# luoao-kddi/SCP

Measured on AMD Instinct MI355X. Metric: KITTI frames/sec encode (SCP-EHEM, level 16) + bpp match vs ref, higher is better.
Workload: dtype f32 (dense layers and attention as bf16x3 split on bf16 MFMA, feature kNN as f16x3 split on f16 MFMA, fp32 accumulate; position kNN / CDF in fp32); 1 GPU; SCP-EHEM KITTI-like synthetic 120k-pt frames, --spher --mullevel lidar_level=16 (BASELINE.json configs[2]), seeded random weights; nodes_per_frame=577403, windows_per_frame=100, frames_per_gpu=46, frames_in_flight=4, frames_per_launch_sequence=1, transform=host-numpy on a prefetch thread (strict identity: the reference's integers), parallelism=frame-sharded x1, rank_cores=256, rank_cores_pinned=False

## Files before the change

### include/scp_debug.h

```cpp
#ifndef SCP_DEBUG_H
#define SCP_DEBUG_H
#include "scp.h"

#ifdef __cplusplus
extern "C" {
#endif

SCP_API int scp_set_knn_mode(int32_t f16x3);
SCP_API int scp_set_attention_mode(int32_t bf16x3);

SCP_API int scp_set_knn_workgroup(int32_t shape);
SCP_API int scp_knn_debug_buffer(unsigned long long *dev_buf);
SCP_API int scp_rc_debug_buffer(unsigned long long *dev_buf);
SCP_API int scp_set_attention_variant(int32_t v);
SCP_API int scp_get_attention_variant(void);
SCP_API int scp_rc_set_grid(int32_t workgroups);
SCP_API int scp_rc_set_wide(int32_t mode);

enum {
    SCP_PROF_POST_ATTN = 1,
    SCP_PROF_LN_LINEAR = 2,
    SCP_PROF_ATTENTION = 3,
    SCP_PROF_KNN_FEAT = 4,
    SCP_PROF_KNN_POS = 5,
    SCP_PROF_GEMM_SPLIT = 6,
    SCP_PROF_EDGE_MLP = 7,
    SCP_PROF_MERGE = 8,
    SCP_PROF_EDGE_GATHER = 9,
    SCP_PROF_CDF = 10,
    SCP_PROF_GEMM_F32 = 11,
    SCP_PROF_GEMM_ROWS = 12,
    SCP_PROF_SPLIT_ROWS = 13,
    SCP_PROF_LAYERNORM = 14,
    SCP_PROF_OA_ATTENTION = 15,
    SCP_PROF_GEOM = 16,
    SCP_PROF_OTHER = 17,
    SCP_PROF_MLP3 = 18,
    SCP_PROF_RATE = 19,
    SCP_PROF_NTAGS = 20
};
SCP_API int scp_prof_enable(int32_t on);
SCP_API int scp_prof_count(void);
SCP_API int scp_prof_read(int32_t cap, int32_t *tags, float *ms, double *work);

#ifdef __cplusplus
// ... 4 lines not shown
```

### scp_amd/csrc/gemm_split.hip

```cpp
#include <stdlib.h>
#include "scp_internal.h"

typedef __bf16 bf16x8 __attribute__((ext_vector_type(8)));
typedef __bf16 bf16x4 __attribute__((ext_vector_type(4)));
typedef _Float16 sf16x8 __attribute__((ext_vector_type(8)));
typedef float f32x16 __attribute__((ext_vector_type(16)));
typedef float f32x4 __attribute__((ext_vector_type(4)));

enum { ACT_NONE = 0, ACT_LEAKY = 1, ACT_GELU = 2, ACT_RELU = 3 };

template <int act>
__device__ __forceinline__ float apply_act_s(float y) {
    if (act == ACT_LEAKY) return y > 0.f ? y : 0.01f * y;
    if (act == ACT_GELU) return scp_gelu(y);
    if (act == ACT_RELU) return y > 0.f ? y : 0.f;
    return y;
}

typedef __attribute__((address_space(3))) void *lds_ptr_t;
typedef const __attribute__((address_space(1))) void *glb_ptr_t;

__device__ __forceinline__ void dma16(const void *g, char *l) {
    __builtin_amdgcn_global_load_lds((glb_ptr_t)g, (lds_ptr_t)l, 16, 0, 0);
}
// ... 567 lines not shown
    const int64_t blk = i >> 6;
    const int nks = Kpad >> 5;
    const int ks = (int)(blk % nks);
    const int64_t rb = blk / nks;
    const int q = p ^ ((r >> 2) & 3);
    dst[i] = src[((rb * 16 + r) * (int64_t)Kpad + 32 * ks + 8 * q) >> 3];
}

extern "C" SCP_API int scp_tile_weight_bf16(const void *plane, int32_t Npad, int32_t Kpad, void *tiled, void *stream) {
    if (!plane || !tiled || Npad <= 0 || Kpad <= 0 || (Npad & 15) || (Kpad & 31) || (((uintptr_t)plane | (uintptr_t)tiled) & 15)) return SCP_EINVAL;
    const int64_t total = (int64_t)Npad * Kpad / 8;
    hipLaunchKernelGGL(tile_weight_kernel, dim3((unsigned)cdiv64(total, 256)), dim3(256), 0, (hipStream_t)stream, (const uint4 *)plane, Npad, Kpad, (uint4 *)tiled);
    LAUNCH_CHECK();
    return SCP_OK;
}

extern "C" SCP_API int scp_split_rows(const float *src, int64_t ld_src, int64_t n_src, const int64_t *idx, int32_t C, void *hi, void *lo,
                                      int64_t ldo, int64_t rows, void *stream) {
    if (!src || !hi || !lo || rows < 0 || C <= 0 || (C & 3) || (ld_src & 3) || (ldo & 7) || ldo < C || (((uintptr_t)src) & 15) ||
        (((uintptr_t)hi | (uintptr_t)lo) & 7))
        return SCP_EINVAL;
    if (rows == 0) return SCP_OK;
    int Cp = (C + 31) & ~31;
    if (Cp > ldo) Cp = C;
    const int64_t total = rows * (Cp / 4);
    SCP_PROF(SCP_PROF_SPLIT_ROWS, stream, 8.0 * rows * C);
    hipLaunchKernelGGL(split_rows_kernel, dim3((unsigned)cdiv64(total, 256)), dim3(256), 0, (hipStream_t)stream, src, ld_src, n_src, idx, C / 4,
                       Cp / 4, (__bf16 *)hi, (__bf16 *)lo, ldo, total);
    LAUNCH_CHECK();
    return SCP_OK;
}

static int g_num_cu = 0;
template <int WM, int WN, int TM, bool EXT, bool F16 = false>
static int launch_cfg(const GemmSplitArgs &ga, int act, hipStream_t st, double work) {
    constexpr int BM = WM * TM * 32, BN = WN * 64;
    constexpr int STAGE = (BM + BN) * 128;
    constexpr int BOUNCE = WM * WN * 8192;
    constexpr int LDS = STAGE + (STAGE > BOUNCE ? STAGE : BOUNCE) + (EXT ? 2 * BM * 8 : 0);
    static bool configured = false;
    if (!configured) {
        HIP_TRY(hipFuncSetAttribute((const void *)gemm_split_kernel<WM, WN, TM, ACT_NONE, EXT, F16>, hipFuncAttributeMaxDynamicSharedMemorySize, LDS));
        HIP_TRY(hipFuncSetAttribute((const void *)gemm_split_kernel<WM, WN, TM, ACT_RELU, EXT, F16>, hipFuncAttributeMaxDynamicSharedMemorySize, LDS));
        if (!F16) {
            HIP_TRY(hipFuncSetAttribute((const void *)gemm_split_kernel<WM, WN, TM, ACT_LEAKY, EXT, false>, hipFuncAttributeMaxDynamicSharedMemorySize, LDS));
            HIP_TRY(hipFuncSetAttribute((const void *)gemm_split_kernel<WM, WN, TM, ACT_GELU, EXT, false>, hipFuncAttributeMaxDynamicSharedMemorySize, LDS));
        }
        configured = true;
    }
    const int64_t ntiles = cdiv64(ga.M, BM) * cdiv64(ga.N, BN);
    const int64_t slots = (int64_t)g_num_cu * (WM * WN == 4 ? 2 : 1);
    const unsigned grid = (unsigned)(ntiles < slots ? ntiles : slots);
    SCP_PROF(SCP_PROF_GEMM_SPLIT, st, work);
#define GOS(ACT, F) hipLaunchKernelGGL((gemm_split_kernel<WM, WN, TM, ACT, EXT, F>), dim3(grid), dim3(WM * WN * 64), LDS, st, ga)
    if (F16) { if (act == ACT_RELU) GOS(ACT_RELU, F16); else GOS(ACT_NONE, F16); }
    else switch (act) { case ACT_LEAKY: GOS(ACT_LEAKY, false); break; case ACT_GELU: GOS(ACT_GELU, false); break; case ACT_RELU: GOS(ACT_RELU, false); break; default: GOS(ACT_NONE, false); }
#undef GOS
    LAUNCH_CHECK();
    return SCP_OK;
}

static int linear_split_impl(const void *Ahi, const void *Alo, int64_t lda, const void *Whi, const void *Wlo, int32_t Npad, int32_t Kpad,
                             const float *bias, const float *residual, int64_t ldr, const int64_t *res_map, int32_t res_first, const int64_t *out_map, float *C, int64_t ldc,
                             void *Ohi, void *Olo, int64_t ldo, int32_t M, int32_t N, int32_t K, int32_t act, int32_t cfg, void *stream) {
    if (!Ahi || !Alo || !Whi || !Wlo || (!C && !Ohi) || ((Ohi == nullptr) != (Olo == nullptr)) || M <= 0 || N <= 0 || K <= 0 || (lda & 7) ||
        Kpad < K || (Kpad & 31) || lda < Kpad || (Npad & 255) || Npad < N || act < 0 || act > 3 || (C && ldc < N) ||
// ... 1 lines not shown
        (((uintptr_t)Ahi | (uintptr_t)Alo | (uintptr_t)Whi | (uintptr_t)Wlo) & 15) || (((uintptr_t)C | (uintptr_t)residual) & 3) ||
        (((uintptr_t)Ohi | (uintptr_t)Olo) & 7))
        return SCP_EINVAL;
    if (!g_num_cu) {
        int dev = 0;
        hipDeviceProp_t p;
        HIP_TRY(hipGetDevice(&dev));
        HIP_TRY(hipGetDeviceProperties(&p, dev));
        g_num_cu = p.multiProcessorCount > 0 ? p.multiProcessorCount : 256;
    }
    GemmSplitArgs ga;
    ga.a_isc = nullptr; ga.w_isc = nullptr; ga.row_max = nullptr; ga.col_max = nullptr; ga.cm_lo = ga.cm_hi = ga.cm_rows = 0;
    ga.Ahi = (const __bf16 *)Ahi; ga.Alo = (const __bf16 *)Alo; ga.lda = lda;
    ga.Whi = (const __bf16 *)Whi; ga.Wlo = (const __bf16 *)Wlo; ga.Kpad = Kpad;
    ga.bias = bias; ga.res = residual; ga.ldr = ldr; ga.C = C; ga.ldc = ldc;
    ga.res_map = residual ? res_map : nullptr; ga.res_first = (residual && res_first) ? 1 : 0;
    ga.out_map = C ? out_map : nullptr;
    ga.Ohi = (__bf16 *)Ohi; ga.Olo = (__bf16 *)Olo; ga.ldo = ldo; ga.M = M; ga.N = N;
    int nco = (N + 31) & ~31;
    if (nco > ldo) nco = (N + 3) & ~3;
    ga.ncols_out = nco;
    { static int wt = -1; if (wt < 0) { const char *e = getenv("SCP_WTILE"); wt = (e && e[0] == '0') ? 0 : 1; } ga.wtiled = wt; }
    if (cfg & ~0xff) {
        static int probe = -1;
        if (probe < 0) probe = getenv("SCP_GEMM_PROBE") ? 1 : 0;
        if (!probe || (cfg & ~0x300ff)) return SCP_EINVAL;
        if (cfg & 0x10000) ga.lda = 0;
        if (cfg & 0x20000) { ga.C = nullptr; ga.Ohi = ga.Olo = nullptr; ga.res = nullptr; }
    }
    cfg &= 255;
    ga.vec_ok = !((C && ((ldc & 3) || ((uintptr_t)C & 15))) || (residual && ((ldr & 3) || ((uintptr_t)residual & 15))));
    hipStream_t st = (hipStream_t)stream;
    const bool ext = ga.res_map || ga.res_first || ga.out_map;
    if (cfg == 0) {
        cfg = (N <= 128) ? 2 : 1;
        static int small = -1;
        if (small < 0) { const char *e = getenv("SCP_GEMM_SMALL"); small = (e && e[0] == '0') ? 0 : 1; }
        if (small && cdiv64(M, 256) * cdiv64(N, 256) * 2 <= g_num_cu) cfg = ext ? 2 : 3;
    }
    const double work = 2.0 * M * (double)N * K;
    if (cfg == 2) return ext ? launch_cfg<4, 2, 2, true>(ga, act, st, work) : launch_cfg<4, 2, 2, false>(ga, act, st, work);
    if (cfg == 3) return ext ? SCP_EINVAL : launch_cfg<2, 2, 2, false>(ga, act, st, work);
    return ext ? launch_cfg<2, 4, 4, true>(ga, act, st, work) : launch_cfg<2, 4, 4, false>(ga, act, st, work);
}

extern "C" SCP_API int scp_linear_split(const void *Ahi, const void *Alo, int64_t lda, const void *Whi, const void *Wlo, int32_t Npad, int32_t Kpad,
                                        const float *bias, const float *residual, int64_t ldr, float *C, int64_t ldc, void *Ohi, void *Olo,
                                        int64_t ldo, int32_t M, int32_t N, int32_t K, int32_t act, int32_t cfg, void *stream) {
    return linear_split_impl(Ahi, Alo, lda, Whi, Wlo, Npad, Kpad, bias, residual, ldr, nullptr, 0, nullptr, C, ldc, Ohi, Olo, ldo, M, N, K, act, cfg, stream);
}

static int linear_split_f16_impl(const void *Ahi, const void *Alo, int64_t lda, const float *a_inv_scale, const void *Whi, const void *Wlo,
                                 const float *w_inv_scale, int32_t Npad, int32_t Kpad, const float *bias, const float *residual, int64_t ldr,
                                 float *C, int64_t ldc, int32_t M, int32_t N, int32_t K, int32_t act, int32_t cfg, uint32_t *row_max, uint32_t *col_max,
                                 int32_t col_lo, int32_t col_hi, int32_t col_rows, void *stream) {
    if (col_max && (col_lo < 0 || col_hi > N || col_lo >= col_hi || col_rows <= 0)) return SCP_EINVAL;
    if ((((uintptr_t)row_max | (uintptr_t)col_max) & 3)) return SCP_EINVAL;
    if (!Ahi || !Alo || !a_inv_scale || !Whi || !Wlo || !w_inv_scale || !C || M <= 0 || N <= 0 || K <= 0 || (lda & 7) || Kpad < K || (Kpad & 31) || cfg < 0 || cfg > 3 ||
        lda < Kpad || (Npad & 255) || Npad < N || (act != ACT_NONE && act != ACT_RELU) || ldc < N || (residual && ldr < N) ||
        (((uintptr_t)Ahi | (uintptr_t)Alo | (uintptr_t)Whi | (uintptr_t)Wlo) & 15) || (((uintptr_t)C | (uintptr_t)residual) & 3))
        return SCP_EINVAL;
    if (!g_num_cu) {
        int dev = 0;
        hipDeviceProp_t p;
        HIP_TRY(hipGetDevice(&dev));
        HIP_TRY(hipGetDeviceProperties(&p, dev));
        g_num_cu = p.multiProcessorCount > 0 ? p.multiProcessorCount : 256;
    }
    GemmSplitArgs ga = {};
    ga.Ahi = (const __bf16 *)Ahi; ga.Alo = (const __bf16 *)Alo; ga.lda = lda;
    ga.Whi = (const __bf16 *)Whi; ga.Wlo = (const __bf16 *)Wlo; ga.Kpad = Kpad;
    ga.bias = bias; ga.res = residual; ga.ldr = ldr; ga.C = C; ga.ldc = ldc; ga.M = M; ga.N = N;
    ga.a_isc = a_inv_scale; ga.w_isc = w_inv_scale;
// ... 82 lines not shown
```

### scp_amd/csrc/knn.hip

```cpp
#include <float.h>
#include <stdlib.h>
#include <limits.h>
#include "scp_internal.h"

#define TK 20
typedef float f32x4 __attribute__((ext_vector_type(4)));
typedef float f32x16 __attribute__((ext_vector_type(16)));

__device__ __forceinline__ void topk_insert(float (&v)[TK], int (&id)[TK], float d, int j) {
#pragma unroll
    for (int t = 0; t < TK; ++t) {
        const bool better = (d > v[t]) || (d == v[t] && j < id[t]);
        const float nv = better ? d : v[t], od = better ? v[t] : d;
        const int ni = better ? j : id[t], oj = better ? id[t] : j;
        v[t] = nv; d = od; id[t] = ni; j = oj;
    }
}

__global__ __launch_bounds__(256) void sqnorm_kernel(const float *__restrict__ x, int64_t npts, int C, float *__restrict__ xx) {
    const int64_t i = (int64_t)blockIdx.x * 256 + threadIdx.x;
    if (i >= npts) return;
    const float *p = x + i * C;
    float s = 0.f;
    for (int c = 0; c < C; ++c) s = s + p[c] * p[c];
// ... 404 lines not shown
        if (s + 2 < nt) { nxt = next_tile(); issue(nxt, (s + 2) % NST); }
        const char *arow = pool + buf * STAGE_B + col * RB;
        f32x16 acc;
#pragma unroll
        for (int r = 0; r < 16; ++r) acc[r] = 0.f;
        f16x8 ca = *(const f16x8 *)(arow + 16 * ((0 + h) ^ swz));
        f16x8 cb = *(const f16x8 *)(arow + 16 * ((K / 8 + h) ^ swz));
        __builtin_amdgcn_sched_group_barrier(0x100, 2, 0);
#pragma unroll
        for (int c = 0; c < NC; ++c) {
            f16x8 na = ca, nb = cb;
            if (c + 1 < NC) {
                na = *(const f16x8 *)(arow + 16 * ((2 * (c + 1) + h) ^ swz));
                nb = *(const f16x8 *)(arow + 16 * ((K / 8 + 2 * (c + 1) + h) ^ swz));
            }
            acc = __builtin_amdgcn_mfma_f32_32x32x16_f16(cb, qa[c], acc, 0, 0, 0);
            acc = __builtin_amdgcn_mfma_f32_32x32x16_f16(ca, qb[c], acc, 0, 0, 0);
            acc = __builtin_amdgcn_mfma_f32_32x32x16_f16(ca, qa[c], acc, 0, 0, 0);
            ca = na; cb = nb;
            if (c + 1 < NC) __builtin_amdgcn_sched_group_barrier(0x100, 2, 0);
            __builtin_amdgcn_sched_group_barrier(0x008, 3, 0);
        }
        const float *sxx = txx + buf * 64;
        knn_select<true>(acc, sxx, sxx + 32, 2.f * isq, xxi, cur * 32, n, h, key, thr0v);
        cur = cur1;
        cur1 = nxt;
    }
    __syncthreads();
    knn_merge_write(key, (float *)pool, (int *)(pool + 128 * 2 * TK * 4), tid, w, col, h, q0, n, k, row0, ctab, idx);
}

struct KnnWg { int32_t row0, n, q0, pad; };

__global__ __launch_bounds__(1024) void knn_sched_kernel(const int *__restrict__ ctab, int nchunks, KnnWg *__restrict__ tab, int nslots, int nspill, int nsplit) {
    __shared__ int seq_base[2048], seq_n[2048], seq_blk0[2049];
    __shared__ unsigned long long seq_w0[2049];
    __shared__ int nseq_s, first_blk[9], spill_s;
    __shared__ unsigned long long wtot_s;
    const int tid = threadIdx.x;
    if (tid == 0) { nseq_s = 0; spill_s = 0; }
    if (tid < 9) first_blk[tid] = INT_MAX;
    __syncthreads();
    if (tid < 64) {
        int cnt = 0;
        for (int g = 0; g < nchunks; g += 64) {
            const int c = g + tid;
            const bool st = c < nchunks && ctab[2 * c] == c * 512 && ctab[2 * c + 1] > 0;
            const unsigned long long m = __ballot(st);
            if (st) {
                const int o = cnt + __popcll(m & ((1ull << tid) - 1ull));
                if (o < 2048) { seq_base[o] = ctab[2 * c]; seq_n[o] = ctab[2 * c + 1]; }
            }
            cnt += __popcll(m);
        }
        if (tid == 0) nseq_s = cnt < 2048 ? cnt : 2048;
    }
    __syncthreads();
    const int nseq = nseq_s;
    if (tid == 0) {
        int b = 0;
        unsigned long long wsum = 0;
        for (int q = 0; q < nseq; ++q) {
            seq_blk0[q] = b; seq_w0[q] = wsum;
            const int nb = ((seq_n[q] + 255) >> 8) * nsplit;
            b += nb; wsum += (unsigned long long)nb * (unsigned)(seq_n[q] / nsplit + 1);
        }
        seq_blk0[nseq] = b; seq_w0[nseq] = wsum; wtot_s = wsum ? wsum : 1ull;
    }
    __syncthreads();
    const int nblk = seq_blk0[nseq];
    const unsigned long long wtot = wtot_s;
    auto xcd_of = [&](int q, int j) { const unsigned long long cw = seq_w0[q] + (unsigned long long)j * (unsigned)(seq_n[q] / nsplit + 1); const int x = (int)(cw * 8ull / wtot); return x > 7 ? 7 : x; };
    for (int q = tid; q < nseq; q += 1024) {
        const int nb = seq_blk0[q + 1] - seq_blk0[q];
        for (int j = 0; j < nb; ++j) atomicMin(&first_blk[xcd_of(q, j)], seq_blk0[q] + j);
    }
    __syncthreads();
    for (int q = tid; q < nseq; q += 1024) {
        const int nb = seq_blk0[q + 1] - seq_blk0[q];
        for (int j = 0; j < nb; ++j) {
            const int x = xcd_of(q, j), slot = seq_blk0[q] + j - first_blk[x];
            KnnWg e; e.row0 = seq_base[q]; e.n = seq_n[q]; e.q0 = (j / nsplit) * 256; e.pad = j % nsplit;
            if (slot < nslots) tab[slot * 8 + x] = e;
            else { const int k = atomicAdd(&spill_s, 1); if (k < nspill) tab[nslots * 8 + k] = e; }
        }
    }
    (void)nblk;
}

template <int K, int G, bool DBG = false>
__global__ __launch_bounds__(512, 2) void knn_f16x3_wg256_kernel(const _Float16 *__restrict__ planes, const float *__restrict__ xx,
                                                                const float *__restrict__ inv_scale, const KnnWg *__restrict__ tab,
                                                                int *__restrict__ idx, const float *__restrict__ thr0, int order,
                                                                unsigned long long *__restrict__ dbg = nullptr, int nsplit = 1,
                                                                float *__restrict__ pval = nullptr, int *__restrict__ pidx = nullptr,
                                                                int64_t prows = 0) {
    constexpr int RB = 4 * K;
    constexpr int R = RB / 16;
    constexpr int NC = K / 16;
    constexpr int STAGE_B = 32 * RB;
    constexpr int NDMA = STAGE_B / 1024;
    constexpr int NDMA_W = (NDMA + 7) / 8;
    constexpr int NST = 2 * G;
    constexpr int NXX = NST;
    constexpr int MERGE_B = 2 * 256 * 2 * TK * 4;
    constexpr int TILES_B = NST * STAGE_B + NXX * 64 * 4;
    constexpr int POOL_B = TILES_B > MERGE_B ? TILES_B : MERGE_B;
    static_assert(STAGE_B % 1024 == 0 && POOL_B <= 160 * 1024, "layout");
    __shared__ __attribute__((aligned(1024))) char pool[POOL_B];
    float *txx = (float *)(pool + NST * STAGE_B);

    const KnnWg wg = tab[blockIdx.x];
    const int n = wg.n;
    if (n <= 0) return;
    const int tid = threadIdx.x, lane = tid & 63, col = lane & 31, h = lane >> 5;
    const int w = __builtin_amdgcn_readfirstlane(tid >> 6);
    const size_t row0 = (size_t)wg.row0;
    const int q0 = wg.q0;
    const char *pb = (const char *)planes + row0 * RB;
    const float *xxb = xx + row0, *isb = inv_scale + row0;
// ... 332 lines not shown

struct KnnScratch { void *stream; bool used; unsigned long long last; DevBuf buf; };
static KnnScratch g_xx_tab[8];
static unsigned long long g_xx_clock = 0;
static DevBuf *knn_scratch(hipStream_t st) {
    ++g_xx_clock;
    for (auto &e : g_xx_tab) if (e.used && e.stream == (void *)st) { e.last = g_xx_clock; return &e.buf; }
    KnnScratch *pick = nullptr;
    for (auto &e : g_xx_tab) if (!e.used) { pick = &e; break; }
    if (!pick) {
        for (auto &e : g_xx_tab) if (!pick || e.last < pick->last) pick = &e;
        pick->buf.release();
    }
    pick->used = true; pick->stream = (void *)st; pick->last = g_xx_clock;
    return &pick->buf;
}

static int g_knn_mode = -1;
static int knn_mode() {
    const int c = scp_ctx_knn_mode();
    if (c >= 0) return c;
    if (g_knn_mode < 0) { const char *e = getenv("SCP_KNN"); g_knn_mode = (e && e[0] == 'f') ? 0 : 1; }
    return g_knn_mode;
}
extern "C" SCP_API int scp_set_knn_mode(int32_t f16x3) { g_knn_mode = f16x3 ? 1 : 0; return SCP_OK; }
static int knn_split_on() {
    static int on = -1;
    if (on < 0) { const char *e = getenv("SCP_KNN_SPLIT"); on = (e && e[0] == '0') ? 0 : 1; }
    return on;
}
static int g_knn_wg = -1;
static int knn_wg() { if (g_knn_wg < 0) { const char *e = getenv("SCP_KNN_WG"); g_knn_wg = e ? atoi(e) : 256; } return g_knn_wg; }
extern "C" SCP_API int scp_set_knn_workgroup(int32_t v) { g_knn_wg = v; return SCP_OK; }

static int knn_launch(const float *x, int64_t npts, int C, dim3 grid, int n, int k, int *idx, const int *ctab, hipStream_t st,
                      const float *thr0 = nullptr) {
    const size_t xx_bytes = ((size_t)npts * sizeof(float) + 1023) & ~(size_t)1023;
    const bool split = (C == 144 || C == 192) && knn_mode() == 1;
    const int RB = C * 4;
    DevBuf *sp = knn_scratch(st);
    if (!sp) return SCP_EINVAL;
    DevBuf &sbuf = *sp;
    int nsplit = 1;
    if (split && ctab && knn_wg() == 256 && !g_knn_dbg && knn_split_on()) {
        const int64_t nblk = npts / 256 > 0 ? npts / 256 : 1;
        while (nsplit < 16 && nblk * (nsplit * 2) <= 256 && npts / 32 >= 8 * (int64_t)nsplit) nsplit *= 2;
    }
    const size_t part_bytes = nsplit > 1 ? (size_t)nsplit * (size_t)npts * TK * 8 + 256 : 0;
    int rc = sbuf.reserve(xx_bytes * (split ? 2 : 1) + (C <= 4 ? (size_t)npts * 16 + ((size_t)npts / 32 + grid.y + 1) * 32 : (split ? (size_t)npts * RB + 256 + (((size_t)(npts / 256) * 2 + 8) * nsplit + 520) * sizeof(KnnWg) + part_bytes : 0)));
    if (rc) return rc;
    float *xx = sbuf.as<float>();
    void *aux = (char *)sbuf.p + xx_bytes;
    if (split) {
        float *isc = (float *)aux;
        _Float16 *pl = (_Float16 *)((char *)aux + xx_bytes);
        hipLaunchKernelGGL(split2_kernel, dim3((unsigned)cdiv64(npts, 64)), dim3(256), 0, st, x, npts, C, pl, xx, isc);
        if (ctab && knn_wg() >= 256 && npts / 512 <= 2048) {
            const int nchunks = (int)(npts / 512);
            const int nspill = (int)(npts / 256) * nsplit;
            const int nslots = nspill / 8 + 64;
            const int nblocks = nslots * 8 + nspill;
            KnnWg *tab = (KnnWg *)((char *)pl + (((size_t)npts * RB + 255) & ~(size_t)255));
            float *pval = (float *)((char *)tab + (((size_t)nblocks * sizeof(KnnWg) + 255) & ~(size_t)255));
            int *pidx = (int *)(pval + (size_t)nsplit * (size_t)npts * TK);
            HIP_TRY(hipMemsetAsync(tab, 0, (size_t)nblocks * sizeof(KnnWg), st));
            hipLaunchKernelGGL(knn_sched_kernel, dim3(1), dim3(1024), 0, st, ctab, nchunks, tab, nslots, nspill, nsplit);
            const int shape = knn_wg() & 15, order = (knn_wg() >> 4) & 7;
            SCP_PROF(SCP_PROF_KNN_FEAT, st, (double)C);
#define KNN_LAUNCH(KK, GG) hipLaunchKernelGGL((knn_f16x3_wg256_kernel<KK, GG>), dim3(nblocks), dim3(512), 0, st, (const _Float16 *)pl, (const float *)xx, \
                                              (const float *)isc, (const KnnWg *)tab, idx, thr0, order, (unsigned long long *)nullptr, nsplit, pval, pidx, (int64_t)npts)
            if (C == 144) { if (shape == 2) KNN_LAUNCH(144, 1); else if (shape == 1) KNN_LAUNCH(144, 2); else KNN_LAUNCH(144, 4); }
            else if (g_knn_dbg && shape == 0)
                hipLaunchKernelGGL((knn_f16x3_wg256_kernel<192, 3, true>), dim3(nblocks), dim3(512), 0, st, (const _Float16 *)pl, (const float *)xx,
                                   (const float *)isc, (const KnnWg *)tab, idx, thr0, order, g_knn_dbg);
            else { if (shape == 2) KNN_LAUNCH(192, 1); else if (shape == 1) KNN_LAUNCH(192, 2); else KNN_LAUNCH(192, 3); }
#undef KNN_LAUNCH
            LAUNCH_CHECK();
            if (nsplit > 1) {
                hipLaunchKernelGGL(knn_merge_split_kernel, dim3((unsigned)cdiv64(npts, 256)), dim3(256), 0, st, ctab, (const float *)pval, (const int *)pidx, (int64_t)npts, nsplit, idx);
                LAUNCH_CHECK();
            }
            return SCP_OK;
        }
        SCP_PROF(SCP_PROF_KNN_FEAT, st, (double)C);
        if (C == 144) hipLaunchKernelGGL(knn_f16x3_kernel<144>, grid, dim3(256), 0, st, (const _Float16 *)pl, (const float *)xx, (const float *)isc, n, k, idx, ctab, thr0);
        else hipLaunchKernelGGL(knn_f16x3_kernel<192>, grid, dim3(256), 0, st, (const _Float16 *)pl, (const float *)xx, (const float *)isc, n, k, idx, ctab, thr0);
        LAUNCH_CHECK();
        return SCP_OK;
    }
    hipLaunchKernelGGL(sqnorm_kernel, dim3((unsigned)cdiv64(npts, 256)), dim3(256), 0, st, x, npts, C, xx);
    if (C <= 4) {
        hipLaunchKernelGGL(pad4_kernel, dim3((unsigned)cdiv64(npts, 256)), dim3(256), 0, st, x, npts, C, (float *)aux);
        float *bb = (float *)((char *)aux + (size_t)npts * 16);
        const int bn = ctab ? (int)npts : n, bB = ctab ? 1 : (int)grid.y;
        hipLaunchKernelGGL(bbox32_kernel, dim3((unsigned)cdiv64((int64_t)((bn + 31) / 32) * bB, 256)), dim3(256), 0, st, (const float *)aux, bn, bB, bb);
        SCP_PROF(SCP_PROF_KNN_POS, st, 4.0);
        hipLaunchKernelGGL((knn_mfma_kernel<2, 16, true>), grid, dim3(256), 0, st, (const float *)aux, (const float *)xx, n, 4, k, idx, ctab, thr0,
                           (const float *)bb);
    } else {
// ... 53 lines not shown
```

### scp_amd/native.py

```python
import ctypes as C
import os

import numpy as np
import torch

HERE = os.path.dirname(os.path.abspath(__file__))
LIB_PATH = os.path.join(HERE, "libscp_hip.so")
MAX_DEPTH = 21

CART, SPHER, CYLIN = 0, 1, 2
POS_MINMAX, POS_MINMAX_MUL, POS_POW2 = 0, 1, 2
_ERR = {-1: "SCP_EINVAL", -2: "SCP_ENOMEM", -3: "SCP_ESMALL", -4: "SCP_EHIP", -5: "SCP_ESTATE"}


class ScpError(RuntimeError):
    pass


class QuantInfo(C.Structure):
    _fields_ = [("bin_num", C.c_double), ("qs", C.c_double * 3), ("offset", C.c_double * 3),
                ("max_coord", C.c_int32), ("min_coord", C.c_int32)]


class Segment(C.Structure):
# ... 45 lines not shown
        "scp_geom_emit_nodes": (C.c_int, [_vp, _vp, _vp, _vp, _vp, _vp, _vp]),
        "scp_geom_emit_leaves": (C.c_int, [_vp, i32, _vp, _vp]),
        "scp_geom_krecords_i64": (C.c_int, [_vp, i32, _vp, _vp]),
        "scp_geom_context_ehem": (C.c_int, [_vp, i32, i32, i32, _vp, _vp, _vp, _vp, _vp]),
        "scp_geom_context_octattn": (C.c_int, [_vp, i32, _vp, _vp, _vp, _vp]),
        "scp_knn_topk": (C.c_int, [_vp, i32, i32, i32, i32, _vp, _vp]),
        "scp_knn_topk_packed": (C.c_int, [_vp, _vp, i32, i32, _vp, _vp]),
        "scp_knn_topk_packed_bounded": (C.c_int, [_vp, _vp, i32, i32, _vp, _vp, _vp]),
        "scp_swin_attention_packed": (C.c_int, [_vp, _vp, _vp, _vp, _vp, i32, i32, i32, i32, _vp, _vp]),
        "scp_swin_attention_packed_split": (C.c_int, [_vp, _vp, _vp, _vp, _vp, i32, i32, i32, i32, _vp, _vp, i64, _vp]),
        "scp_set_attention_mode": (C.c_int, [i32]),
        "scp_set_attention_variant": (C.c_int, [i32]),
        "scp_get_attention_variant": (C.c_int, []),
        "scp_ctx_create": (C.c_int, [C.POINTER(_vp)]),
        "scp_ctx_destroy": (C.c_int, [_vp]),
        "scp_ctx_set": (C.c_int, [_vp, i32, i32]),
        "scp_ctx_get": (C.c_int, [_vp, i32]),
        "scp_ctx_make_current": (C.c_int, [_vp]),
        "scp_rc_debug_buffer": (C.c_int, [_vp]),
        "scp_rc_set_wide": (C.c_int, [i32]),
        "scp_prof_enable": (C.c_int, [i32]),
        "scp_prof_count": (C.c_int, []),
        "scp_prof_read": (C.c_int, [i32, _vp, _vp, _vp]),
        "scp_set_knn_mode": (C.c_int, [i32]),
        "scp_row_scale_f16": (C.c_int, [_vp, i64, i32, i32, _vp, _vp, _vp]),
        "scp_row_scale_from_max": (C.c_int, [_vp, i32, _vp, _vp, _vp]),
        "scp_linear_split_f16_max": (C.c_int, [_vp, _vp, i64, _vp, _vp, _vp, _vp, i32, i32, _vp, _vp, i64, _vp, i64, i32, i32, i32, i32, i32, _vp, _vp, i32, i32, i32, _vp]),
        "scp_octattn_attention_f16x3_vmax": (C.c_int, [_vp, _vp, _vp, _vp, _vp, i64, i32, i32, i32, i32, _vp, _vp, _vp, i64, _vp, _vp]),
        "scp_linear_f16x3_scaled": (C.c_int, [_vp, i64, _vp, _vp, _vp, i32, _vp, _vp, i64, _vp, i64, i32, i32, i32, i32, _vp, _vp, _vp]),
        "scp_layernorm_add": (C.c_int, [_vp, _vp, i64, i32, _vp, _vp, C.c_float, _vp, _vp]),
        "scp_layernorm_add_split_f16": (C.c_int, [_vp, _vp, i64, i32, _vp, _vp, C.c_float, _vp, _vp, _vp, i64, _vp, _vp, _vp]),
        "scp_set_knn_workgroup": (C.c_int, [i32]),
        "scp_knn_debug_buffer": (C.c_int, [_vp]),
        "scp_nn_sqdist_f64": (C.c_int, [_vp, i64, _vp, i64, _vp, _vp]),
        "scp_estimate_normals_f64": (C.c_int, [_vp, i64, C.c_double, i32, _vp, _vp, _vp, _vp, _vp]),
        "scp_nn_tieset_f64": (C.c_int, [i32, _vp, i64, _vp, i64, _vp, _vp, _vp, _vp]),
        "scp_edge_gather_max_ld": (C.c_int, [_vp, i64, _vp, i64, _vp, _vp, _vp, i32, i32, i32, i32, _vp, i32, _vp]),
        "scp_embed_gather": (C.c_int, [_vp, _vp, _vp, i64, _vp, _vp, _vp, _vp, _vp, _vp, i64, _vp]),
        "scp_packed_plan_sizes": (C.c_int, [_vp, i32, _vp]),
        "scp_packed_plan": (C.c_int, [_vp, i32, _vp, _vp, i32, _vp]),
        "scp_decode_expand": (C.c_int, [_vp, _vp, _vp, _vp, _vp, i64, i32, i32, i32, i32, i32, C.c_double, C.c_double, _vp, _vp, _vp, _vp, _vp, _vp, _vp]),
        "scp_edge_gather_max": (C.c_int, [_vp, _vp, _vp, _vp, _vp, i32, i32, i32, i32, _vp, i32, _vp]),
        "scp_swin_attention": (C.c_int, [_vp, _vp, _vp, _vp, i32, i32, i32, i32, i32, _vp, _vp]),
        "scp_octattn_attention": (C.c_int, [_vp, _vp, _vp, _vp, _vp, i32, i32, i32, i32, _vp, _vp, _vp]),
        "scp_octattn_f16x3_ws_bytes": (C.c_int64, [i32, i32, i32]),
        "scp_octattn_embed": (C.c_int, [_vp, _vp, i64, i32, _vp, i32, _vp, i32, i32, _vp, i32, _vp, _vp, i32, _vp, i32, _vp, _vp, _vp, i64, _vp, _vp, _vp]),
        "scp_octattn_attention_f16x3": (C.c_int, [_vp, _vp, _vp, _vp, _vp, i64, i32, i32, i32, i32, _vp, _vp, _vp, i64, _vp]),
        "scp_octattn_attention_rowinv": (C.c_int, [_vp, i64, i64, _vp, _vp, i64, i64, _vp, _vp, i64, i64, _vp, _vp, i64, i64, i32, i32, i32, i32, i32,
                                                   i32, _vp]),
        "scp_octattn_attention_rowinv_step": (C.c_int, [_vp, i64, _vp, _vp, i64, i64, i32, i32, _vp, _vp, i64, _vp, _vp, i64, _vp, _vp, i32, i32, i32,
                                                        _vp]),
        "scp_decode_expand_octattn": (C.c_int, [_vp, _vp, _vp, _vp, i64, i32, i32, i32, _vp, _vp, _vp, _vp, _vp]),
        "scp_decode_expand_batch": (C.c_int, [_vp, _vp, _vp, _vp, _vp, i64, _vp, i32, i32, _vp, i32, i64, i64, _vp, _vp, _vp, _vp, _vp, _vp, _vp, _vp]),
        "scp_split_weight_bf16": (C.c_int, [_vp, i32, i32, i32, i32, _vp, _vp, _vp]),
        "scp_linear_bf16x3": (C.c_int, [_vp, i64, _vp, _vp, i32, _vp, _vp, i64, _vp, i64, i32, i32, i32, i32, _vp]),
        "scp_split_weight_f16": (C.c_int, [_vp, i32, i32, i32, i32, _vp, _vp, _vp, _vp]),
        "scp_linear_f16x3": (C.c_int, [_vp, i64, _vp, _vp, _vp, i32, _vp, _vp, i64, _vp, i64, i32, i32, i32, i32, _vp, _vp]),
        "scp_linear_split": (C.c_int, [_vp, _vp, i64, _vp, _vp, i32, i32, _vp, _vp, i64, _vp, i64, _vp, _vp, i64, i32, i32, i32, i32, i32, _vp]),
        "scp_tile_weight_bf16": (C.c_int, [_vp, i32, i32, _vp, _vp]),
        "scp_swin_ln_linear": (C.c_int, [_vp, i64, _vp, _vp, _vp, _vp, _vp, C.c_float, _vp, i64, i32, i32, _vp]),
        "scp_swin_post_attn": (C.c_int, [_vp, _vp, i64, _vp, i64, _vp, _vp, _vp, _vp, C.c_float, _vp, i64, i32, _vp, i32, _vp]),
        "scp_swin_post_attn_weight_bytes": (C.c_int64, []),
        "scp_gelu_prescale": (C.c_double, []),
        "scp_split_rows": (C.c_int, [_vp, i64, i64, _vp, i32, _vp, _vp, i64, i64, _vp]),
        "scp_linear_split_scatter": (C.c_int, [_vp, _vp, i64, _vp, _vp, i32, i32, _vp, _vp, _vp, i64, i32, i32, i32, i32, i32, _vp]),
        "scp_linear_split_gather": (C.c_int, [_vp, _vp, i64, _vp, _vp, i32, i32, _vp, _vp, i64, _vp, _vp, i64, _vp, _vp, i64, i32, i32, i32, i32, i32, _vp]),
# ... 483 lines not shown
            L = (L + 1) // 2
        return out
    parts = lists(e, n_self) + lists(e // 2, n_cross)
    flat = torch.from_numpy(np.concatenate(parts)).to(device, non_blocking=True)
    cuts = np.cumsum([0] + [len(p) for p in parts])
    views = [flat[cuts[i]:cuts[i + 1]] for i in range(len(parts))]
    return views[:n_self], views[n_self:]


def edge_gather_max_rows(u, v, idx, scale, shift, out=None):
    n, Co = u.shape
    if out is None:
        out = torch.empty((n, Co), dtype=torch.float32, device=u.device)
    elif out.shape != (n, Co) or out.stride(1) != 1 or out.dtype != torch.float32 or out.stride(0) % 4 or out.data_ptr() % 16:
        raise ScpError("edge_gather_max_rows: out must be a float32 [n, C'] view with unit channel stride and 16-byte aligned rows")
    _check(lib().scp_edge_gather_max_ld(u.data_ptr(), u.stride(0), v.data_ptr(), v.stride(0), _dev(idx, torch.int32), _dev(scale), _dev(shift),
                                        1, n, Co, idx.shape[1], out.data_ptr(), out.stride(0), _stream()), "scp_edge_gather_max_ld")
    return out


_MODES = {"knn": "f32" if os.environ.get("SCP_KNN", "")[:1] == "f" else "f16x3",
          "attn": "f32" if os.environ.get("SCP_ATTN", "")[:1] == "f" else "bf16x3"}


def set_knn_mode(f16x3):
    _check(lib().scp_set_knn_mode(1 if f16x3 else 0), "scp_set_knn_mode")
    _MODES["knn"] = "f16x3" if f16x3 else "f32"


def set_knn_workgroup(shape):
    _check(lib().scp_set_knn_workgroup(int(shape)), "scp_set_knn_workgroup")


class NumericProfile:

    def __init__(self, knn_f16x3=True, attention_bf16x3=True):
        self._h = _vp()
        _check(lib().scp_ctx_create(C.byref(self._h)), "scp_ctx_create")
        self.knn_f16x3, self.attention_bf16x3 = bool(knn_f16x3), bool(attention_bf16x3)
        _check(lib().scp_ctx_set(self._h, 1, int(self.knn_f16x3)), "scp_ctx_set")
        _check(lib().scp_ctx_set(self._h, 2, int(self.attention_bf16x3)), "scp_ctx_set")

    def describe(self, model_name):
        return numeric_profile(model_name, self)

    def __del__(self):
        try:
            if self._h:
                lib().scp_ctx_destroy(self._h)
        except Exception:
            pass


_TLS = __import__("threading").local()


def current_profile():
    return getattr(_TLS, "profile", None)


class use_profile:

    def __init__(self, profile):
        self.profile = profile

    def __enter__(self):
# ... 1379 lines not shown
```

Baseline: 15.83 frames/s.

## Balance kNN block schedule across XCDs and split GEMM leftover wave tiles

The kNN scheduler kernel now builds a second, greedy longest-first placement of 32-block units across the 8 XCDs. It simulates the makespan of both the contiguous-cut and the aligned tables on device and keeps whichever is shorter, and spill slots are now assigned deterministically per XCD. Separately, the split GEMM auto-config peels off a partial last wave of 256x256 tiles into a second launch with a smaller tile config, so the tail uses more CUs. The cost is extra scheduler work, an extra launch, and more scratch memory, plus a debug API to read the schedule table.

```diff
diff --git a/include/scp_debug.h b/include/scp_debug.h
--- a/include/scp_debug.h
+++ b/include/scp_debug.h
@@ -11,6 +11,7 @@
 
 SCP_API int scp_set_knn_workgroup(int32_t shape);
 SCP_API int scp_knn_debug_buffer(unsigned long long *dev_buf);
+SCP_API int scp_knn_sched_table(int32_t cap, int32_t *entries, int32_t *info);
 SCP_API int scp_rc_debug_buffer(unsigned long long *dev_buf);
 SCP_API int scp_set_attention_variant(int32_t v);
 SCP_API int scp_get_attention_variant(void);
diff --git a/scp_amd/csrc/gemm_split.hip b/scp_amd/csrc/gemm_split.hip
--- a/scp_amd/csrc/gemm_split.hip
+++ b/scp_amd/csrc/gemm_split.hip
@@ -623,6 +623,7 @@
 }
 
 static int g_num_cu = 0;
+#define LEFTOVER_SHARE 4
 template <int WM, int WN, int TM, bool EXT, bool F16 = false>
 static int launch_cfg(const GemmSplitArgs &ga, int act, hipStream_t st, double work) {
     constexpr int BM = WM * TM * 32, BN = WN * 64;
@@ -690,6 +691,7 @@
     ga.vec_ok = !((C && ((ldc & 3) || ((uintptr_t)C & 15))) || (residual && ((ldr & 3) || ((uintptr_t)residual & 15))));
     hipStream_t st = (hipStream_t)stream;
     const bool ext = ga.res_map || ga.res_first || ga.out_map;
+    const bool auto_cfg = cfg == 0;
     if (cfg == 0) {
         cfg = (N <= 128) ? 2 : 1;
         static int small = -1;
@@ -697,6 +699,24 @@
         if (small && cdiv64(M, 256) * cdiv64(N, 256) * 2 <= g_num_cu) cfg = ext ? 2 : 3;
     }
     const double work = 2.0 * M * (double)N * K;
+    if (auto_cfg && cfg == 1 && !ext) {
+        static int leftover = -1;
+        if (leftover < 0) { const char *e = getenv("SCP_GEMM_LEFTOVER"); leftover = (e && e[0] == '0') ? 0 : 1; }
+        const int64_t tn = cdiv64(N, 256), nt = cdiv64(M, 256) * tn;
+        const int64_t rounds = nt / g_num_cu, rem = nt % g_num_cu;
+        if (leftover && rounds >= 1 && rem > 0 && rem * LEFTOVER_SHARE <= g_num_cu) {
+            const int64_t M1 = rounds * g_num_cu / tn * 256;
+            GemmSplitArgs g1 = ga, g2 = ga;
+            g1.M = (int)M1; g2.M = (int)(M - M1);
+            g2.Ahi = ga.Ahi + M1 * ga.lda; g2.Alo = ga.Alo + M1 * ga.lda;
+            if (ga.res) g2.res = ga.res + M1 * ga.ldr;
+            if (ga.C) g2.C = ga.C + M1 * ga.ldc;
+            if (ga.Ohi) { g2.Ohi = ga.Ohi + M1 * ga.ldo; g2.Olo = ga.Olo + M1 * ga.ldo; }
+            g2.vec_ok = ga.vec_ok && !(ga.C && ((uintptr_t)g2.C & 15)) && !(ga.res && ((uintptr_t)g2.res & 15));
+            const int rc = launch_cfg<2, 4, 4, false>(g1, act, st, work * (double)M1 / M);
+            return rc ? rc : launch_cfg<2, 2, 2, false>(g2, act, st, work * (double)(M - M1) / M);
+        }
+    }
     if (cfg == 2) return ext ? launch_cfg<4, 2, 2, true>(ga, act, st, work) : launch_cfg<4, 2, 2, false>(ga, act, st, work);
     if (cfg == 3) return ext ? SCP_EINVAL : launch_cfg<2, 2, 2, false>(ga, act, st, work);
     return ext ? launch_cfg<2, 4, 4, true>(ga, act, st, work) : launch_cfg<2, 4, 4, false>(ga, act, st, work);
diff --git a/scp_amd/csrc/knn.hip b/scp_amd/csrc/knn.hip
--- a/scp_amd/csrc/knn.hip
+++ b/scp_amd/csrc/knn.hip
@@ -460,14 +460,64 @@
 
 struct KnnWg { int32_t row0, n, q0, pad; };
 
-__global__ __launch_bounds__(1024) void knn_sched_kernel(const int *__restrict__ ctab, int nchunks, KnnWg *__restrict__ tab, int nslots, int nspill, int nsplit) {
+#ifndef KNN_BLOCK_CONST
+#define KNN_BLOCK_CONST 28
+#endif
+#define KNN_SCHED_MAXU 2304
+enum { KNN_SCHED_CUT = 0, KNN_SCHED_ALIGNED = 1, KNN_SCHED_AUTO = 2 };
+
+__device__ __forceinline__ int knn_entry_cost(int n, int part, int nsplit) {
+    const int nt_all = (n + 31) >> 5;
+    const int nt = nsplit > 1 ? (int)((int64_t)nt_all * (part + 1) / nsplit) - (int)((int64_t)nt_all * part / nsplit) : nt_all;
+    return nt + KNN_BLOCK_CONST;
+}
+
+__device__ int knn_sched_eval(const KnnWg *tab, int x, int nslots, int nspill, int nsplit, int lane) {
+    int f = lane < 32 ? 0 : INT_MAX;
+    const int npos = nslots + (nspill > x ? (nspill - x + 7) / 8 : 0);
+    for (int p0 = 0; p0 < npos; p0 += 64) {
+        const int p = p0 + lane;
+        int cost = 0;
+        if (p < npos) {
+            const KnnWg e = p < nslots ? tab[p * 8 + x] : tab[nslots * 8 + (p - nslots) * 8 + x];
+            if (e.n > 0) cost = knn_entry_cost(e.n, e.pad, nsplit);
+        }
+        unsigned long long m = __ballot(cost > 0);
+#pragma unroll
+        for (int half = 0; half < 2; ++half) {
+            const unsigned hm = (unsigned)(m >> (32 * half));
+            const int c0 = __builtin_amdgcn_readlane(cost, 32 * half);
+            const bool same = hm == 0xffffffffu && (unsigned)(__ballot(cost == c0) >> (32 * half)) == 0xffffffffu;
+            if (same && (half == 0 || (unsigned)m == 0u) && c0 >= __builtin_amdgcn_readlane(f, 31) - __builtin_amdgcn_readfirstlane(f)) {
+                if (lane < 32) f += c0;
+                m &= ~(0xffffffffull << (32 * half));
+            }
+        }
+        while (m) {
+            const int b = __ffsll((long long)m) - 1;
+            m &= m - 1;
+            const int v = __builtin_amdgcn_readfirstlane(f) + __builtin_amdgcn_readlane(cost, b);
+            const int up = __shfl_down(f, 1);
+            const int k = __popcll(__ballot(lane >= 1 && lane < 32 && f <= v));
+            if (lane < 32) f = lane < k ? up : (lane == k ? v : f);
+        }
+    }
+    return __builtin_amdgcn_readlane(f, 31);
+}
+
+__global__ __launch_bounds__(1024) void knn_sched_kernel(const int *__restrict__ ctab, int nchunks, KnnWg *tab, KnnWg *tab2, int *info,
+                                                          int nslots, int nspill, int nsplit, int mode) {
     __shared__ int seq_base[2048], seq_n[2048], seq_blk0[2049];
+    __shared__ unsigned short seq_u0[2048];
     __shared__ unsigned long long seq_w0[2049];
-    __shared__ int nseq_s, first_blk[9], spill_s;
+    __shared__ int nseq_s, first_blk[9], spill_base[8], nunit_s, mk_s[16];
     __shared__ unsigned long long wtot_s;
+    __shared__ unsigned short unit_seq[KNN_SCHED_MAXU], unit_j0[KNN_SCHED_MAXU], unit_sorted[KNN_SCHED_MAXU];
+    __shared__ unsigned unit_key[KNN_SCHED_MAXU], unit_place[KNN_SCHED_MAXU];
     const int tid = threadIdx.x;
-    if (tid == 0) { nseq_s = 0; spill_s = 0; }
+    if (tid == 0) { nseq_s = 0; nunit_s = 0; }
     if (tid < 9) first_blk[tid] = INT_MAX;
+    if (tid < 16) mk_s[tid] = 0;
     __syncthreads();
     if (tid < 64) {
         int cnt = 0;
@@ -486,22 +536,32 @@
     __syncthreads();
     const int nseq = nseq_s;
     if (tid == 0) {
-        int b = 0;
+        int b = 0, nu = 0;
         unsigned long long wsum = 0;
         for (int q = 0; q < nseq; ++q) {
-            seq_blk0[q] = b; seq_w0[q] = wsum;
+            seq_blk0[q] = b; seq_w0[q] = wsum; seq_u0[q] = (unsigned short)nu;
             const int nb = ((seq_n[q] + 255) >> 8) * nsplit;
-            b += nb; wsum += (unsigned long long)nb * (unsigned)(seq_n[q] / nsplit + 1);
-        }
-        seq_blk0[nseq] = b; seq_w0[nseq] = wsum; wtot_s = wsum ? wsum : 1ull;
-    }
-    __syncthreads();
-    const int nblk = seq_blk0[nseq];
+            b += nb; wsum += (unsigned long long)nb * (unsigned)(seq_n[q] / nsplit + 1); nu += (nb + 31) >> 5;
+        }
+        seq_blk0[nseq] = b; seq_w0[nseq] = wsum; wtot_s = wsum ? wsum : 1ull; nunit_s = nu < KNN_SCHED_MAXU ? nu : KNN_SCHED_MAXU;
+    }
+    __syncthreads();
     const unsigned long long wtot = wtot_s;
     auto xcd_of = [&](int q, int j) { const unsigned long long cw = seq_w0[q] + (unsigned long long)j * (unsigned)(seq_n[q] / nsplit + 1); const int x = (int)(cw * 8ull / wtot); return x > 7 ? 7 : x; };
     for (int q = tid; q < nseq; q += 1024) {
         const int nb = seq_blk0[q + 1] - seq_blk0[q];
         for (int j = 0; j < nb; ++j) atomicMin(&first_blk[xcd_of(q, j)], seq_blk0[q] + j);
+    }
+    __syncthreads();
+    if (tid == 0) {
+        int sp = 0;
+        for (int x = 0; x < 8; ++x) {
+            int nxt = seq_blk0[nseq];
+            for (int y = 7; y > x; --y) if (first_blk[y] != INT_MAX) nxt = first_blk[y];
+            const int len = first_blk[x] == INT_MAX ? 0 : nxt - first_blk[x];
+            spill_base[x] = sp;
+            sp += len > nslots ? len - nslots : 0;
+        }
     }
     __syncthreads();
     for (int q = tid; q < nseq; q += 1024) {
@@ -510,10 +570,77 @@
             const int x = xcd_of(q, j), slot = seq_blk0[q] + j - first_blk[x];
             KnnWg e; e.row0 = seq_base[q]; e.n = seq_n[q]; e.q0 = (j / nsplit) * 256; e.pad = j % nsplit;
             if (slot < nslots) tab[slot * 8 + x] = e;
-            else { const int k = atomicAdd(&spill_s, 1); if (k < nspill) tab[nslots * 8 + k] = e; }
-        }
-    }
-    (void)nblk;
+            else { const int k = spill_base[x] + slot - nslots; if (k < nspill) tab[nslots * 8 + k] = e; }
+        }
+    }
+    if (mode == KNN_SCHED_CUT) { if (tid == 0) info[0] = KNN_SCHED_CUT; return; }
+
+    const int nu = nunit_s;
+    for (int q = tid; q < nseq; q += 1024) {
+        const int nb = seq_blk0[q + 1] - seq_blk0[q];
+        int u = seq_u0[q];
+        for (int j0 = 0; j0 < nb && u < KNN_SCHED_MAXU; j0 += 32, ++u) {
+            unit_seq[u] = (unsigned short)q; unit_j0[u] = (unsigned short)j0;
+            const int cnt = nb - j0 < 32 ? nb - j0 : 32;
+            unit_key[u] = ((unsigned)seq_n[q] << 6) | (unsigned)cnt;
+        }
+    }
+    __syncthreads();
+    for (int u = tid; u < nu; u += 1024) {
+        const unsigned ku = unit_key[u];
+        int r = 0;
+        for (int v = 0; v < nu; ++v) { const unsigned kv = unit_key[v]; r += (kv > ku || (kv == ku && v < u)) ? 1 : 0; }
+        unit_sorted[r] = (unsigned short)u;
+    }
+    __syncthreads();
+    if (tid == 0) {
+        unsigned load[8], cn[8];
+#pragma unroll
+        for (int x = 0; x < 8; ++x) { load[x] = 0; cn[x] = 0; }
+        for (int i = 0; i < nu; ++i) {
+            const int u = unit_sorted[i];
+            const unsigned key = unit_key[u], cnt = key & 63u;
+            const unsigned cost = cnt * (unsigned)knn_entry_cost((int)(key >> 6), 0, nsplit);
+            int bx = 0; unsigned bl = load[0];
+#pragma unroll
+            for (int x = 1; x < 8; ++x) if (load[x] < bl) { bl = load[x]; bx = x; }
+            unsigned s0 = 0;
+#pragma unroll
+            for (int x = 0; x < 8; ++x) if (x == bx) { s0 = cn[x]; cn[x] += cnt; load[x] += cost; }
+            unit_place[u] = (unsigned)bx | (s0 << 3);
+        }
+        unsigned sp = 0;
+#pragma unroll
+        for (int x = 0; x < 8; ++x) { spill_base[x] = (int)sp; sp += cn[x] > (unsigned)nslots ? cn[x] - (unsigned)nslots : 0u; }
+    }
+    __syncthreads();
+    for (int u = tid; u < nu; u += 1024) {
+        const int q = unit_seq[u], j0 = unit_j0[u], cnt = (int)(unit_key[u] & 63u);
+        const int x = (int)(unit_place[u] & 7u), s0 = (int)(unit_place[u] >> 3);
+        for (int i = 0; i < cnt; ++i) {
+            const int j = j0 + i, slot = s0 + i;
+            KnnWg e; e.row0 = seq_base[q]; e.n = seq_n[q]; e.q0 = (j / nsplit) * 256; e.pad = j % nsplit;
+            if (slot < nslots) tab2[slot * 8 + x] = e;
+            else { const int k = spill_base[x] + slot - nslots; if (k < nspill) tab2[nslots * 8 + k] = e; }
+        }
+    }
+    __syncthreads();
+
+    {
+        const int w = tid >> 6, lane = tid & 63;
+        const int mk = knn_sched_eval(w < 8 ? tab : tab2, w & 7, nslots, nspill, nsplit, lane);
+        if (lane == 0) mk_s[w] = mk;
+    }
+    __syncthreads();
+    int mk_cut = 0, mk_al = 0;
+    for (int x = 0; x < 8; ++x) { mk_cut = mk_s[x] > mk_cut ? mk_s[x] : mk_cut; mk_al = mk_s[8 + x] > mk_al ? mk_s[8 + x] : mk_al; }
+    const bool aligned = mode == KNN_SCHED_ALIGNED || mk_al < mk_cut;
+    if (tid == 0) { info[0] = aligned ? KNN_SCHED_ALIGNED : KNN_SCHED_CUT; info[1] = mk_cut; info[2] = mk_al; info[3] = nu; info[4] = nseq; }
+    if (aligned) {
+        const int4 *src = (const int4 *)tab2;
+        int4 *dst = (int4 *)tab;
+        for (int i = tid; i < nslots * 8 + nspill; i += 1024) dst[i] = src[i];
+    }
 }
 
 template <int K, int G, bool DBG = false>
@@ -912,6 +1039,23 @@
 static int g_knn_wg = -1;
 static int knn_wg() { if (g_knn_wg < 0) { const char *e = getenv("SCP_KNN_WG"); g_knn_wg = e ? atoi(e) : 256; } return g_knn_wg; }
 extern "C" SCP_API int scp_set_knn_workgroup(int32_t v) { g_knn_wg = v; return SCP_OK; }
+static int knn_sched_mode() {
+    static int m = -1;
+    if (m < 0) { const char *e = getenv("SCP_KNN_SCHED"); m = (e && e[0] == 'c') ? KNN_SCHED_CUT : (e && e[0] == 'a' && e[1] == 'l') ? KNN_SCHED_ALIGNED : KNN_SCHED_AUTO; }
+    return m;
+}
+static struct { const KnnWg *tab; const int *info; int nblocks, nslots, nspill, nsplit; hipStream_t st; } g_knn_last = {nullptr, nullptr, 0, 0, 0, 0, nullptr};
+extern "C" SCP_API int scp_knn_sched_table(int32_t cap, int32_t *entries, int32_t *info) {
+    if (!g_knn_last.tab || !info || (cap > 0 && !entries)) return SCP_EINVAL;
+    HIP_TRY(hipStreamSynchronize(g_knn_last.st));
+    int32_t dev[8];
+    HIP_TRY(hipMemcpy(dev, g_knn_last.info, sizeof(dev), hipMemcpyDeviceToHost));
+    info[0] = g_knn_last.nslots; info[1] = g_knn_last.nspill; info[2] = g_knn_last.nsplit; info[3] = dev[0]; info[4] = dev[1]; info[5] = dev[2];
+    info[6] = knn_sched_mode(); info[7] = KNN_BLOCK_CONST;
+    const int n = cap < g_knn_last.nblocks ? cap : g_knn_last.nblocks;
+    if (n > 0) HIP_TRY(hipMemcpy(entries, g_knn_last.tab, (size_t)n * sizeof(KnnWg), hipMemcpyDeviceToHost));
+    return g_knn_last.nblocks;
+}
 
 static int knn_launch(const float *x, int64_t npts, int C, dim3 grid, int n, int k, int *idx, const int *ctab, hipStream_t st,
                       const float *thr0 = nullptr) {
@@ -927,7 +1071,7 @@
         while (nsplit < 16 && nblk * (nsplit * 2) <= 256 && npts / 32 >= 8 * (int64_t)nsplit) nsplit *= 2;
     }
     const size_t part_bytes = nsplit > 1 ? (size_t)nsplit * (size_t)npts * TK * 8 + 256 : 0;
-    int rc = sbuf.reserve(xx_bytes * (split ? 2 : 1) + (C <= 4 ? (size_t)npts * 16 + ((size_t)npts / 32 + grid.y + 1) * 32 : (split ? (size_t)npts * RB + 256 + (((size_t)(npts / 256) * 2 + 8) * nsplit + 520) * sizeof(KnnWg) + part_bytes : 0)));
+    int rc = sbuf.reserve(xx_bytes * (split ? 2 : 1) + (C <= 4 ? (size_t)npts * 16 + ((size_t)npts / 32 + grid.y + 1) * 32 : (split ? (size_t)npts * RB + 256 + 2 * (((size_t)(npts / 256) * 2 + 8) * nsplit + 520) * sizeof(KnnWg) + part_bytes : 0)));
     if (rc) return rc;
     float *xx = sbuf.as<float>();
     void *aux = (char *)sbuf.p + xx_bytes;
@@ -941,10 +1085,13 @@
             const int nslots = nspill / 8 + 64;
             const int nblocks = nslots * 8 + nspill;
             KnnWg *tab = (KnnWg *)((char *)pl + (((size_t)npts * RB + 255) & ~(size_t)255));
-            float *pval = (float *)((char *)tab + (((size_t)nblocks * sizeof(KnnWg) + 255) & ~(size_t)255));
+            KnnWg *tab2 = tab + nblocks;
+            int *sinfo = (int *)(tab2 + nblocks);
+            float *pval = (float *)((char *)tab + (((size_t)(2 * nblocks + 2) * sizeof(KnnWg) + 255) & ~(size_t)255));
             int *pidx = (int *)(pval + (size_t)nsplit * (size_t)npts * TK);
-            HIP_TRY(hipMemsetAsync(tab, 0, (size_t)nblocks * sizeof(KnnWg), st));
-            hipLaunchKernelGGL(knn_sched_kernel, dim3(1), dim3(1024), 0, st, ctab, nchunks, tab, nslots, nspill, nsplit);
+            HIP_TRY(hipMemsetAsync(tab, 0, (size_t)(2 * nblocks + 2) * sizeof(KnnWg), st));
+            hipLaunchKernelGGL(knn_sched_kernel, dim3(1), dim3(1024), 0, st, ctab, nchunks, tab, tab2, sinfo, nslots, nspill, nsplit, knn_sched_mode());
+            g_knn_last = {tab, sinfo, nblocks, nslots, nspill, nsplit, st};
             const int shape = knn_wg() & 15, order = (knn_wg() >> 4) & 7;
             SCP_PROF(SCP_PROF_KNN_FEAT, st, (double)C);
 #define KNN_LAUNCH(KK, GG) hipLaunchKernelGGL((knn_f16x3_wg256_kernel<KK, GG>), dim3(nblocks), dim3(512), 0, st, (const _Float16 *)pl, (const float *)xx, \
diff --git a/scp_amd/native.py b/scp_amd/native.py
--- a/scp_amd/native.py
+++ b/scp_amd/native.py
@@ -101,6 +101,7 @@
         "scp_layernorm_add_split_f16": (C.c_int, [_vp, _vp, i64, i32, _vp, _vp, C.c_float, _vp, _vp, _vp, i64, _vp, _vp, _vp]),
         "scp_set_knn_workgroup": (C.c_int, [i32]),
         "scp_knn_debug_buffer": (C.c_int, [_vp]),
+        "scp_knn_sched_table": (C.c_int, [i32, _vp, _vp]),
         "scp_nn_sqdist_f64": (C.c_int, [_vp, i64, _vp, i64, _vp, _vp]),
         "scp_estimate_normals_f64": (C.c_int, [_vp, i64, C.c_double, i32, _vp, _vp, _vp, _vp, _vp]),
         "scp_nn_tieset_f64": (C.c_int, [i32, _vp, i64, _vp, i64, _vp, _vp, _vp, _vp]),
@@ -650,6 +651,15 @@
     _check(lib().scp_set_knn_workgroup(int(shape)), "scp_set_knn_workgroup")
 
 
+def knn_sched_table():
+    info = np.zeros(8, np.int32)
+    n = _check(lib().scp_knn_sched_table(0, None, info.ctypes.data), "scp_knn_sched_table")
+    ent = np.zeros((n, 4), np.int32)
+    _check(lib().scp_knn_sched_table(n, ent.ctypes.data, info.ctypes.data), "scp_knn_sched_table")
+    keys = ("nslots", "nspill", "nsplit", "chosen", "makespan_cut", "makespan_aligned", "mode", "block_const")
+    return ent, dict(zip(keys, (int(v) for v in info)))
+
+
 class NumericProfile:
 
     def __init__(self, knn_f16x3=True, attention_bf16x3=True):
```

Result: no change. 15.69 frames/s (-0.9%).
